# iamgroot42/A-LINK

Measured on AMD Instinct MI355X. Metric: 112x112 face embeddings/sec (IR-ResNet-100 ArcFace, 512-d, L2-normalised), higher is better.
Workload: dtype bf16

## Files before the change

### a-link_amd/csrc/alink_common.h

```cpp
#pragma once
#include <hip/hip_runtime.h>
#include <stdint.h>
#include <stddef.h>
#include <string>

#include "../../include/alink_hip.h"
#include "conv_kernel.h"

namespace alink {

void set_error(const char* fmt, ...);
int  hip_fail(hipError_t e, const char* what, const char* file, int line);

#define ALINK_HIP(call)                                                          \
    do {                                                                         \
        hipError_t e__ = (call);                                                 \
        if (e__ != hipSuccess) return ::alink::hip_fail(e__, #call, __FILE__, __LINE__); \
    } while (0)

#define ALINK_REQUIRE(cond, code, ...)          \
    do {                                        \
        if (!(cond)) {                          \
            ::alink::set_error(__VA_ARGS__);    \
            return (code);                      \
        }                                       \
    } while (0)

static inline int current_device() {
    int d = -1;
    return hipGetDevice(&d) == hipSuccess ? d : -1;
}
static inline int device_of_pointer(const void* p) {
    if (p) {
        hipPointerAttribute_t a;
        if (hipPointerGetAttributes(&a, p) == hipSuccess && a.type == hipMemoryTypeDevice) return a.device;
        (void)hipGetLastError();
    }
    return current_device();
}
struct DeviceGuard {
    int prev = -1;
    bool switched = false;
    explicit DeviceGuard(int dev) {
        if (dev < 0 || hipGetDevice(&prev) != hipSuccess || prev == dev) return;
        switched = hipSetDevice(dev) == hipSuccess;
    }
    ~DeviceGuard() {
        if (switched) (void)hipSetDevice(prev);
    }
    DeviceGuard(const DeviceGuard&) = delete;
    DeviceGuard& operator=(const DeviceGuard&) = delete;
};

typedef __attribute__((ext_vector_type(8))) __bf16   bf16x8;
typedef __attribute__((ext_vector_type(8))) _Float16 f16x8;
typedef __attribute__((ext_vector_type(4))) float    f32x4;
typedef __attribute__((ext_vector_type(16))) float   f32x16;

struct ConvParams {
    const void*  in;
    const void*  wgt;
    const float* bias;
    const float* alpha;
    const void*  resid;
    const void*  dact;
    void*        out;
    const void*  zero;
    const void*  in2;
    int Cin2;
    int in2_compact;
    int N, H, W, Cin, Cout, Ho, Wo, stride, ksz, pad, M;
    int border_cls;
    int splitk;
    int ksteps_per_split;
    int post_relu;
    int fine;
    int stagger;
    int ablate;
    float acc_scale;
    float bias_scale;
    float res_scale;
    int nprod;
    void* stamps;
};

hipError_t launch_conv_igemm(int dtype, const ConvParams& p, hipStream_t stream);
double     conv_flops(const ConvParams& p);

struct StemParams {
    const void*  in;
    const void*  wgt;
    const float* bias;
    const float* alpha;
    void*        out;
    int N, H, W, C0, layout;
    float sub[3], mul;
    int flip;
    float acc_scale, bias_scale;
};
hipError_t launch_stem(int dtype, const StemParams& p, hipStream_t stream);

struct FcFinishParams {
    const float* slabs;
    const float* bias;
    float*       out;
    float*       norms;
    int S, M, E;
    float scale;
    int*  nonfinite;
};
hipError_t launch_fc_finish(const FcFinishParams& p, hipStream_t stream);
hipError_t launch_absmax_f16(const void* x, size_t n_elements, unsigned* out_bits, hipStream_t stream);
hipError_t launch_conv_split_finish(int dtype, const ConvParams& p, const float* slabs, int S, hipStream_t stream);

ConvKernel direct_variant(int ksz, int stride, int pad, int H, int W, int Cin, int Cout);
ConvKernel direct_variant_tiles(int ksz, int stride, int pad, int H, int W, int Cin, int Cout);
ConvKernel linear_variant_x2(int ksz, int stride, int pad, int H, int W, int Cin, int Cout);
hipError_t launch_conv(ConvKernel k, int dtype, const ConvParams& p, hipStream_t st);
hipError_t direct_set_attributes();
ConvKernel linear_variant(int ksz, int stride, int pad, int H, int W, int Cin, int Cout);
ConvKernel c64_variant(int ksz, int stride, int pad, int H, int W, int Cin, int Cout);
ConvKernel s2c64_variant(int ksz, int stride, int pad, int H, int W, int Cin, int Cout);
hipError_t launch_conv3x3_linear(ConvKernel k, int dtype, const ConvParams& p, hipStream_t st);
hipError_t launch_conv3x3_c64(int dtype, const ConvParams& p, hipStream_t st);
hipError_t launch_conv3x3_s2c64(int dtype, const ConvParams& p, hipStream_t st);
hipError_t c64_set_attributes();
hipError_t s2c64_set_attributes();
bool       s2c64_enabled();
hipError_t linear_set_attributes();
hipError_t linear_check_contract();
bool       front_c64_applies(int dtype, int H, int W, int C0, int Cout);
hipError_t front_c64_set_attributes();
hipError_t launch_front_c64(int dtype, const ConvParams& conv1, const StemParams& stem, void* xs, bool slopes_le_1, hipStream_t st);
bool       unit_c64_applies(int dtype, const ConvParams& c1, const ConvParams& c2);
hipError_t unit_c64_set_attributes();
hipError_t launch_unit_c64(int dtype, const ConvParams& c1, const ConvParams& c2, hipStream_t st);
bool       unit1_c64_applies(int dtype, const ConvParams& c1, const StemParams& stem, const ConvParams& c2);
int        unit1_c64_mode();
hipError_t unit1_c64_set_attributes();
hipError_t launch_unit1_c64(int dtype, const ConvParams& c1, const StemParams& stem, const ConvParams& c2, bool slopes_le_1, hipStream_t st);
bool       conv3x3_lat_applies(int dtype, const ConvParams& p);
hipError_t launch_conv3x3_lat(int dtype, const ConvParams& p, hipStream_t stream);
bool       conv_gemm_lat_applies(int dtype, const ConvParams& p);
hipError_t launch_conv_gemm_lat(int dtype, const ConvParams& p, hipStream_t stream);

hipError_t launch_l2norm_bwd(int dtype, const float* g, const float* e, const float* norms, void* dz, int M, int E,
                             hipStream_t st);
hipError_t launch_zero_insert(int dtype, const void* in, void* out, int N, int H, int W, int Ho, int Wo, int C,
                              hipStream_t st);
hipError_t launch_stem_bwd(int dtype, const void* dy0, const void* y0, const float* w, const float* alpha, float* dpix,
                           int N, int H, int W, float mul, int nchw, hipStream_t st);

hipError_t launch_r50_grad_scale(const float* dfeat, int count, int HW, float* scale, hipStream_t st);
hipError_t launch_r50_avgpool_bwd(int dtype, const float* dfeat, const void* y, void* dz, const float* scale, int N, int HW, int C,
                                  hipStream_t st);
hipError_t launch_r50_relu_mask(int dtype, void* g, const void* y, long long count, hipStream_t st);
hipError_t launch_r50_scatter_mask(int dtype, const void* in, const void* y, void* out, int N, int H, int W, int Ho, int Wo, int C,
                                   hipStream_t st);
hipError_t launch_r50_maxpool_bwd(int dtype, const void* y0, const void* pooled, const void* g, void* d0, int N, int H, int W, int C,
                                  int Hp, int Wp, hipStream_t st);
hipError_t launch_r50_stem_bwd(int dtype, const void* d0, const void* wfrag, float* dpix, const float* scale, int N, int H, int W,
                               int Ho, int Wo, int pad_t, int pad_l, int flip, hipStream_t st);
int r50_stem_bwd_max_width();

uint16_t f32_to_bf16_rne(float f);
uint16_t f32_to_f16_rne(float f);

int init_kernels();

__device__ __forceinline__ float relu_keep_nan(float v) { return v < 0.f ? 0.f : v; }
__device__ __forceinline__ float max_keep_nan(float a, float b) { return (a < b || b != b) ? b : a; }

}
#include <map>
#include <string>
#include <vector>
namespace alink {
struct F32Net;
F32Net* f32net_build(const std::map<std::string, std::vector<float>>& raw, const alink_ir_cfg& cfg);
void    f32net_destroy(F32Net* n);
size_t  f32net_workspace_bytes(const F32Net* n, int N);
int     f32net_embed(const F32Net* n, const void* dev_in, int layout, int N, float* dev_out, void* ws, size_t ws_bytes,
                     hipStream_t st);

}
```

### a-link_amd/csrc/conv3x3_linear.hip

```cpp
#include "conv_device.h"

namespace alink {
namespace {

template <int A>
struct IC { static constexpr int a = A; };

constexpr int GPX = 224;
constexpr int TPW = 7;
constexpr int NT = 256;

template <int W, int TCW>
struct Lin {
    static constexpr int BN = 2 * TCW * 16;
    static constexpr int XPIX = GPX + 2 * W + 2;
    static constexpr int XSLOTS = (XPIX * 8 + NT - 1) / NT;
    static constexpr int XBYTES = XSLOTS * NT * 16;
    static constexpr int WOFF = XBYTES;
    static constexpr int WBYTES = BN * 128;
    static constexpr size_t lds_bytes() { return (size_t)WOFF + 2 * WBYTES + 10 * BN * 4; }
    static_assert(GPX % W == 0, "a workgroup covers whole rows");
};

template <typename T, int W, int TCW, int EPI, bool SP, int NP = 3>
__global__ __launch_bounds__(NT, 2) void conv3x3_linear_kernel(const ConvParams p) {
    typedef typename Vec8<T>::type vec8;
    typedef Lin<W, TCW> G;
    constexpr int BN = G::BN, XSLOTS = G::XSLOTS, WBYTES = G::WBYTES, WSLOTS = BN * 8 / NT;
    extern __shared__ __attribute__((aligned(16))) char smem[];

    const int tid = threadIdx.x, lane = tid & 63;
    const int wave = __builtin_amdgcn_readfirstlane(tid >> 6);
    const int wpx = wave >> 1, wco = wave & 1;
    if (p.stagger > 0) {
        __shared__ int s_late;
        if (tid == 0) s_late = (int)(__builtin_amdgcn_s_getreg(6148) & 1u);
        __syncthreads();
        if (s_late)
            for (int i = 0; i < p.stagger; ++i) __builtin_amdgcn_s_sleep(16);
    }
    const int q = lane >> 4, lr = lane & 15;
    const int H = p.H, Cin = p.Cin;
    unsigned long long* const stamps = (EPI == 1 || EPI == 2) ? nullptr : (unsigned long long*)p.stamps;
    unsigned long long refill_cycles = 0;
    if (stamps && tid == 0) stamps[(size_t)blockIdx.x * 8 + 0] = __builtin_amdgcn_s_memtime();
    constexpr int NPH = SP ? NP : 1;
    const int CinP = SP ? 2 * Cin : Cin;
    const int ncc_all = Cin >> 6;
    const int ncc = ncc_all / p.splitk, cc_first = (int)blockIdx.y * ncc;
    const int nk = ncc * 9 * NPH;
    const int K = 9 * CinP;
    const long long totpix = (long long)p.N * H * W;

    const int ntn = p.Cout / BN;
    const int lid = xcd_remap(blockIdx.x, gridDim.x);
    const int tile_n = lid % ntn, grp = lid / ntn;
    const int n0 = tile_n * BN;
    const long long gp0 = (long long)grp * GPX;

    const T* __restrict__ gin = (const T*)p.in;
    const T* __restrict__ gw = (const T*)p.wgt;
    const T* __restrict__ gz = (const T*)p.zero;

    const int xpos0 = tid >> 3;
    const int xc16 = (tid & 7) ^ ((tid >> 4) & 7);
    const long long xgp0 = gp0 - W - 1 + xpos0;
    auto stage_x = [&](int cc, int part = 0) {
        long long x0 = xgp0;
        if (SP) asm volatile("" : "+v"(x0));
#pragma unroll
        for (int i = 0; i < XSLOTS; ++i) {
            const long long gp = x0 + 32 * i;
            const bool ok = xpos0 + 32 * i < G::XPIX && gp >= 0 && gp < totpix;
            const T* src = ok ? gin + ((size_t)gp * CinP + (SP ? 2 * cc + part : cc) * 64 + xc16 * 8) : gz + (lane & 7) * 8;
            dma16(src, smem + (NT * i + wave * 64) * 16);
        }
    };
    const unsigned woff0 = (unsigned)((tid >> 3) * K + (((tid & 7) ^ ((tid >> 4) & 7)) * 8));
    const T* wstep = gw + (size_t)n0 * K + (size_t)cc_first * (SP ? 18 : 9) * 64;
    int wr = 0;
    auto stage_w = [&](int bufoff) {
#pragma unroll
        for (int i = 0; i < WSLOTS; ++i)
            dma16(wstep + (woff0 + (unsigned)(32 * i * K)), smem + G::WOFF + bufoff + (NT * i + wave * 64) * 16);
        if (SP && NP == 1) {
            wstep += wr == 8 ? 10 * 64 : 64;
            wr = wr == 8 ? 0 : wr + 1;
        } else if (SP) {
            wstep += wr == 17 ? -17 * 64 : (wr == 26 ? 10 * 64 : 64);
            wr = wr == 26 ? 0 : wr + 1;
        } else {
            wstep += 64;
        }
    };

    stage_x(cc_first);
    stage_w(0);
    const int ncls = p.border_cls ? 9 : 1;
    constexpr int TBL_TRIPS = (9 * BN + NT - 1) / NT;
    static_assert(BN <= NT, "the slope table is one trip");
    float tbias[TBL_TRIPS], talpha;
#pragma unroll
    for (int k = 0; k < TBL_TRIPS; ++k) {
        const int i = tid + NT * k;
        tbias[k] = p.bias[i < ncls * BN ? (i / BN) * p.Cout + n0 + (i % BN) : 0];
    }
    {
        const float* ap = p.alpha ? p.alpha + n0 + (tid < BN ? tid : 0) : p.bias;
        talpha = *ap;
    }

    const int dl = delta(lr);
    const int xbase = wpx * (TPW * 2048);
    unsigned border = 0;
#pragma unroll
    for (int u = 0; u < TPW; ++u) {
        const int pl = 16 * (wpx * TPW + u) + dl;
        const int col = pl % W;
        const int y = (int)(((unsigned)grp * (unsigned)(GPX / W) + (unsigned)(pl / W)) % (unsigned)W);
        border |= ((y == 0 ? 1u : 0u) | (y == H - 1 ? 2u : 0u) | (col == 0 ? 4u : 0u) | (col == W - 1 ? 8u : 0u)) << (4 * u);
    }
    int wl[2];
    {
        const int rowb = wco * (16 * TCW) + lr;
        const int f = (lr >> 1) & 7;
        wl[0] = G::WOFF + rowb * 128 + (((0 | q) ^ f) << 4);
        wl[1] = G::WOFF + rowb * 128 + (((4 | q) ^ f) << 4);
    }

    f32x4 acc[TCW][TPW];
#pragma unroll
    for (int t = 0; t < TCW; ++t)
#pragma unroll
        for (int u = 0; u < TPW; ++u) acc[t][u] = f32x4{0.f, 0.f, 0.f, 0.f};

    asm volatile("" : "+v"(border));
#pragma unroll
    for (int t = 0; t < TCW; ++t)
#pragma unroll
        for (int u = 0; u < TPW; ++u) asm volatile("" : "+v"(acc[t][u]));

    float* const ebias = (float*)(smem + G::WOFF + 2 * WBYTES);
    float* const ealpha = ebias + 9 * BN;
#pragma unroll
    for (int k = 0; k < TBL_TRIPS; ++k) {
        const int i = tid + NT * k;
        if (i < ncls * BN) ebias[i] = tbias[k] * (SP ? p.bias_scale : 1.f);
    }
    if (p.alpha && tid < BN) ealpha[tid] = talpha;
    wait_then_barrier<0>();
    if (stamps && tid == 0) stamps[(size_t)blockIdx.x * 8 + 1] = __builtin_amdgcn_s_memtime();

    int wtog = 0;
    for (int cc = 0; cc < ncc; ++cc) {
#pragma unroll 1
      for (int ph = 0; ph < NPH; ++ph) {
        auto step = [&](auto tapc) {
            constexpr int tap = decltype(tapc)::a;
            constexpr int ky = tap / 3, kx = tap % 3;
            constexpr unsigned tapbits = (ky == 0 ? 1u : 0u) | (ky == 2 ? 2u : 0u) | (kx == 0 ? 4u : 0u) | (kx == 2 ? 8u : 0u);
            const int t = (cc * NPH + ph) * 9 + tap;
            if (t + 1 < nk) stage_w(wtog ^ WBYTES);
            unsigned bnow = border;
            int sdl = dl;
            asm volatile("" : "+v"(bnow), "+v"(sdl));
            const int spos = sdl + ky * W + kx;
            const int xt0 = xbase + spos * 128 + ((q ^ ((spos >> 1) & 7)) << 4);
            const int xt1 = xt0 ^ 64;
#pragma unroll
            for (int ks = 0; ks < 2; ++ks) {
                vec8 wf[TCW], pf[TPW];
#pragma unroll
                for (int tt = 0; tt < TCW; ++tt) wf[tt] = *(const vec8*)(smem + (wl[ks] + wtog) + tt * 2048);
#pragma unroll
                for (int u = 0; u < TPW; ++u) {
                    const unsigned t = tapbits ? (bnow & (tapbits << (4 * u))) : 0u;
                    const unsigned far = 4 * u < 18 ? t << (18 - (4 * u < 18 ? 4 * u : 0)) : t;
                    pf[u] = *(const vec8*)(smem + ((ks ? xt1 : xt0) + (int)far) + 2048 * u);
                }
#pragma unroll
                for (int tt = 0; tt < TCW; ++tt)
#pragma unroll
                    for (int u = 0; u < TPW; ++u) acc[tt][u] = mfma16<T>(wf[tt], pf[u], acc[tt][u]);
            }
            wait_then_barrier<0>();
            wtog ^= WBYTES;
        };
        step(IC<0>{}); step(IC<1>{}); step(IC<2>{});
        step(IC<3>{}); step(IC<4>{}); step(IC<5>{});
        step(IC<6>{}); step(IC<7>{}); step(IC<8>{});
        const bool next_chunk = ph == NPH - 1;
        if (next_chunk ? cc + 1 < ncc : ph == 1) {
            const unsigned long long t0 = stamps ? __builtin_amdgcn_s_memtime() : 0ull;
            if (next_chunk) stage_x(cc_first + cc + 1, 0);
            else            stage_x(cc_first + cc, 1);
            wait_then_barrier<0>();
            if (stamps) refill_cycles += __builtin_amdgcn_s_memtime() - t0;
        }
      }
    }
    if (stamps && tid == 0) {
        stamps[(size_t)blockIdx.x * 8 + 2] = __builtin_amdgcn_s_memtime();
        stamps[(size_t)blockIdx.x * 8 + 4] = refill_cycles;
        stamps[(size_t)blockIdx.x * 8 + 5] = (unsigned long long)(ncc - 1);
    }

    constexpr int CPL = TCW * 4;
    const int wbase = wco * (16 * TCW);
    auto chan_t = [&](int t) { return wbase + (TCW == 4 ? 32 * (t >> 1) + 8 * q + 4 * (t & 1) : 8 * q + 4 * t); };
    auto chan_h = [&](int h) { return wbase + (TCW == 4 ? 32 * h + 8 * q : 8 * q); };
    if (SP ? EPI == 3 : (EPI == 0 && p.splitk > 1)) {
        float* slab = (float*)p.out + (size_t)blockIdx.y * (size_t)totpix * p.Cout;
#pragma unroll
        for (int u = 0; u < TPW; ++u) {
            const long long gp = gp0 + 16 * (wpx * TPW + u) + dl;
            if (gp < totpix) {
#pragma unroll
                for (int t = 0; t < TCW; ++t) *(f32x4*)(slab + (size_t)gp * p.Cout + n0 + chan_t(t)) = acc[t][u];
            }
        }
        return;
    }
    if constexpr (SP) {
        size_t off[TPW];
        bool ok[TPW];
#pragma unroll
        for (int u = 0; u < TPW; ++u) {
            const long long gp = gp0 + 16 * (wpx * TPW + u) + dl;
            ok[u] = gp < totpix;
            off[u] = (size_t)(ok[u] ? gp : 0) * (2 * p.Cout);
            const unsigned b4 = (border >> (4 * u)) & 15u;
            const int rc = (b4 & 1u) ? 0 : ((b4 & 2u) ? 2 : 1);
            const int ccl = (b4 & 4u) ? 0 : ((b4 & 8u) ? 2 : 1);
            const int cls = p.border_cls ? rc * 3 + ccl : 0;
#pragma unroll
            for (int t = 0; t < TCW; ++t) {
                const f32x4 b = *(const f32x4*)(ebias + cls * BN + chan_t(t));
#pragma unroll
                for (int j = 0; j < 4; ++j) acc[t][u][j] = fmaf(acc[t][u][j], p.acc_scale, b[j]);
            }
        }
        if (EPI == 1 || (EPI == 0 && p.alpha)) {
#pragma unroll
            for (int t = 0; t < TCW; ++t) {
                const f32x4 a4 = *(const f32x4*)(ealpha + chan_t(t));
#pragma unroll
                for (int u = 0; u < TPW; ++u)
#pragma unroll
                    for (int j = 0; j < 4; ++j) acc[t][u][j] = acc[t][u][j] > 0.f ? acc[t][u][j] : acc[t][u][j] * a4[j];
            }
        }
        int so[CPL / 8];
#pragma unroll
        for (int h = 0; h < CPL / 8; ++h) so[h] = ((n0 + chan_h(h)) >> 6) * 128 + ((n0 + chan_h(h)) & 63);
        if (EPI != 1 && p.resid) {
            const T* r = (const T*)p.resid;
#pragma unroll
            for (int part = 0; part < 2; ++part) {
                vec8 res[TPW][CPL / 8];
#pragma unroll
                for (int u = 0; u < TPW; ++u)
#pragma unroll
                    for (int h = 0; h < CPL / 8; ++h) res[u][h] = *(const vec8*)(r + off[u] + so[h] + 64 * part);
#pragma unroll
                for (int u = 0; u < TPW; ++u)
#pragma unroll
                    for (int h = 0; h < CPL / 8; ++h)
#pragma unroll
                        for (int i = 0; i < 8; ++i)
                            acc[2 * h + (i >> 2)][u][i & 3] = fmaf((float)res[u][h][i], p.res_scale, acc[2 * h + (i >> 2)][u][i & 3]);
            }
        }
#pragma unroll
        for (int u = 0; u < TPW; ++u) {
            if (!ok[u]) continue;
#pragma unroll
            for (int h = 0; h < CPL / 8; ++h) {
                vec8 o8, l8;
#pragma unroll
                for (int i = 0; i < 8; ++i) {
                    float v = acc[2 * h + (i >> 2)][u][i & 3];
                    if (EPI == 0 && p.post_relu) v = relu_keep_nan(v);
                    o8[i] = (T)v;
                    l8[i] = (T)(v - (float)o8[i]);
                }
                *(vec8*)((T*)p.out + off[u] + so[h]) = o8;
                *(vec8*)((T*)p.out + off[u] + so[h] + 64) = l8;
            }
        }
        return;
    }
    auto epilogue16 = [&](auto fullc) {
        constexpr bool FULL = decltype(fullc)::a != 0;
        size_t off[TPW];
        bool ok[TPW];
        int cls[TPW];
#pragma unroll
        for (int u = 0; u < TPW; ++u) {
            const long long gp = gp0 + 16 * (wpx * TPW + u) + dl;
            ok[u] = FULL || gp < totpix;
            off[u] = (size_t)(FULL || ok[u] ? gp : 0) * p.Cout + n0;
            const unsigned b4 = (border >> (4 * u)) & 15u;
            const int rc = (b4 & 1u) ? 0 : ((b4 & 2u) ? 2 : 1);
            const int ccl = (b4 & 4u) ? 0 : ((b4 & 8u) ? 2 : 1);
            cls[u] = p.border_cls ? rc * 3 + ccl : 0;
        }
        vec8 res[TPW][CPL / 8];
        const T* extra = EPI == 1 ? (const T*)nullptr : (const T*)((EPI == 0 && p.dact) ? p.dact : p.resid);
        if (EPI == 2 || (EPI == 0 && extra)) {
#pragma unroll
            for (int u = 0; u < TPW; ++u)
#pragma unroll
                for (int h = 0; h < CPL / 8; ++h) res[u][h] = *(const vec8*)(extra + off[u] + chan_h(h));
            __builtin_amdgcn_sched_barrier(0);
        }
        if (stamps) {
            asm volatile("s_waitcnt vmcnt(0)" ::: "memory");
            if (tid == 0) stamps[(size_t)blockIdx.x * 8 + 6] = __builtin_amdgcn_s_memtime();
        }
#pragma unroll
        for (int u = 0; u < TPW; ++u) {
            float v[CPL];
#pragma unroll
            for (int t = 0; t < TCW; ++t) {
                const f32x4 b4 = *(const f32x4*)(ebias + cls[u] * BN + chan_t(t));
#pragma unroll
                for (int j = 0; j < 4; ++j) v[4 * t + j] = acc[t][u][j] + b4[j];
            }
            if (EPI == 0 && p.dact) {
#pragma unroll
                for (int t = 0; t < TCW; ++t) {
                    const f32x4 a4 = *(const f32x4*)(ealpha + chan_t(t));
#pragma unroll
                    for (int j = 0; j < 4; ++j) v[4 * t + j] *= (float)res[u][(4 * t + j) / 8][(4 * t + j) % 8] > 0.f ? 1.f : a4[j];
                }
            } else {
                if (EPI == 1 || (EPI == 0 && p.alpha)) {
#pragma unroll
                    for (int t = 0; t < TCW; ++t) {
                        const f32x4 a4 = *(const f32x4*)(ealpha + chan_t(t));
#pragma unroll
                        for (int j = 0; j < 4; ++j) v[4 * t + j] = v[4 * t + j] > 0.f ? v[4 * t + j] : v[4 * t + j] * a4[j];
                    }
                }
                if (EPI == 2 || (EPI == 0 && p.resid)) {
#pragma unroll
                    for (int h = 0; h < CPL / 8; ++h)
#pragma unroll
                        for (int i = 0; i < 8; ++i) v[8 * h + i] += (float)res[u][h][i];
                }
            }
            if (EPI == 0 && p.post_relu) {
#pragma unroll
                for (int i = 0; i < CPL; ++i) v[i] = relu_keep_nan(v[i]);
            }
            if (FULL || ok[u]) {
#pragma unroll
                for (int h = 0; h < CPL / 8; ++h) {
                    vec8 o8;
#pragma unroll
                    for (int i = 0; i < 8; ++i) o8[i] = (T)v[8 * h + i];
                    *(vec8*)((T*)p.out + off[u] + chan_h(h)) = o8;
                }
            }
        }
    };
    if (gp0 + GPX <= totpix) epilogue16(IC<1>{});
    else                     epilogue16(IC<0>{});
    if (stamps && tid == 0) {
        stamps[(size_t)blockIdx.x * 8 + 7] = __builtin_amdgcn_s_memtime();
        asm volatile("s_waitcnt vmcnt(0)" ::: "memory");
        stamps[(size_t)blockIdx.x * 8 + 3] = __builtin_amdgcn_s_memtime();
    }
}

bool g_generic_epilogue = false;

template <typename T, int W, int TCW, bool SP = false>
hipError_t launch_one(const ConvParams& p, hipStream_t st) {
    typedef Lin<W, TCW> G;
    const long long totpix = (long long)p.N * p.H * W;
    const long long groups = (totpix + GPX - 1) / GPX;
    const long long nwg = groups * (p.Cout / G::BN);
    if (nwg <= 0 || nwg >= (1ll << 31)) return hipErrorInvalidValue;
    const dim3 grid((unsigned)nwg, (unsigned)p.splitk);
    if (SP) {
        if (p.dact) return hipErrorInvalidValue;
        if (p.nprod == 1) {
            if (p.splitk > 1) hipLaunchKernelGGL((conv3x3_linear_kernel<T, W, TCW, 3, SP, 1>), grid, dim3(NT), G::lds_bytes(), st, p);
            else              hipLaunchKernelGGL((conv3x3_linear_kernel<T, W, TCW, 0, SP, 1>), grid, dim3(NT), G::lds_bytes(), st, p);
            return hipGetLastError();
        }
        const bool plain_sp = p.splitk == 1 && !p.post_relu && !p.stamps && !g_generic_epilogue;
        if (p.splitk > 1) hipLaunchKernelGGL((conv3x3_linear_kernel<T, W, TCW, 3, SP>), grid, dim3(NT), G::lds_bytes(), st, p);
        else if (plain_sp && p.alpha && !p.resid)
            hipLaunchKernelGGL((conv3x3_linear_kernel<T, W, TCW, 1, SP>), grid, dim3(NT), G::lds_bytes(), st, p);
        else if (plain_sp && !p.alpha && p.resid)
            hipLaunchKernelGGL((conv3x3_linear_kernel<T, W, TCW, 2, SP>), grid, dim3(NT), G::lds_bytes(), st, p);
        else              hipLaunchKernelGGL((conv3x3_linear_kernel<T, W, TCW, 0, SP>), grid, dim3(NT), G::lds_bytes(), st, p);
        return hipGetLastError();
    }
    const bool plain = p.splitk == 1 && !p.dact && !p.post_relu && !p.stamps && !g_generic_epilogue;
    if (plain && p.alpha && !p.resid)
        hipLaunchKernelGGL((conv3x3_linear_kernel<T, W, TCW, 1, false>), grid, dim3(NT), G::lds_bytes(), st, p);
    else if (plain && !p.alpha && p.resid)
        hipLaunchKernelGGL((conv3x3_linear_kernel<T, W, TCW, 2, false>), grid, dim3(NT), G::lds_bytes(), st, p);
    else
        hipLaunchKernelGGL((conv3x3_linear_kernel<T, W, TCW, 0, false>), grid, dim3(NT), G::lds_bytes(), st, p);
    return hipGetLastError();
}
template <typename T, int W, int TCW>
hipError_t set_attr_one() {
    const int lds = (int)Lin<W, TCW>::lds_bytes();
    hipError_t e = hipFuncSetAttribute((const void*)conv3x3_linear_kernel<T, W, TCW, 0, false>, hipFuncAttributeMaxDynamicSharedMemorySize, lds);
    if (e == hipSuccess) e = hipFuncSetAttribute((const void*)conv3x3_linear_kernel<T, W, TCW, 1, false>, hipFuncAttributeMaxDynamicSharedMemorySize, lds);
    if (e == hipSuccess) e = hipFuncSetAttribute((const void*)conv3x3_linear_kernel<T, W, TCW, 2, false>, hipFuncAttributeMaxDynamicSharedMemorySize, lds);
    return e;
}
template <int W, int TCW>
hipError_t set_attr_sp() {
    hipError_t e = hipFuncSetAttribute((const void*)conv3x3_linear_kernel<_Float16, W, TCW, 0, true>,
                                       hipFuncAttributeMaxDynamicSharedMemorySize, (int)Lin<W, TCW>::lds_bytes());
    if (e == hipSuccess)
        e = hipFuncSetAttribute((const void*)conv3x3_linear_kernel<_Float16, W, TCW, 3, true>,
                                hipFuncAttributeMaxDynamicSharedMemorySize, (int)Lin<W, TCW>::lds_bytes());
    if (e == hipSuccess)
        e = hipFuncSetAttribute((const void*)conv3x3_linear_kernel<_Float16, W, TCW, 1, true>,
                                hipFuncAttributeMaxDynamicSharedMemorySize, (int)Lin<W, TCW>::lds_bytes());
    if (e == hipSuccess)
        e = hipFuncSetAttribute((const void*)conv3x3_linear_kernel<_Float16, W, TCW, 2, true>,
                                hipFuncAttributeMaxDynamicSharedMemorySize, (int)Lin<W, TCW>::lds_bytes());
    if (e == hipSuccess)
        e = hipFuncSetAttribute((const void*)conv3x3_linear_kernel<_Float16, W, TCW, 0, true, 1>,
                                hipFuncAttributeMaxDynamicSharedMemorySize, (int)Lin<W, TCW>::lds_bytes());
    if (e == hipSuccess)
        e = hipFuncSetAttribute((const void*)conv3x3_linear_kernel<_Float16, W, TCW, 3, true, 1>,
                                hipFuncAttributeMaxDynamicSharedMemorySize, (int)Lin<W, TCW>::lds_bytes());
    return e;
}

int g_linear_mode = 31;

}

extern "C" void alink_debug_set_linear(int mode) { g_linear_mode = mode; }
extern "C" void alink_debug_set_generic_epilogue(int on) { g_generic_epilogue = on != 0; }

namespace {
__global__ void lds_oob_probe_kernel(float* out) {
    __shared__ __attribute__((aligned(16))) float buf[256];
    for (int i = threadIdx.x; i < 256; i += 64) buf[i] = 1.0f + i;
    __syncthreads();
    const unsigned base = (unsigned)(size_t)(__attribute__((address_space(3))) float*)buf;
    const int lane = threadIdx.x;
    unsigned bits;
    if (lane < 10) {
        bits = 1u << (18 + lane);
    } else if (lane < 55) {
        int k = lane - 10, a = 18;
        while (k >= 27 - a) { k -= 27 - a; ++a; }
        bits = (1u << a) | (1u << (a + 1 + k));
    } else {
        bits = 0x0FFC0000u >> (lane - 55) & 0x0FFC0000u;
    }
    const unsigned far = base + (lane & 15) * 16u + bits, near = base + (lane & 3) * 16u;
    f32x4 a0, a1, b;
    asm volatile("ds_read_b128 %0, %3\n\tds_read_b128 %1, %3 offset:12288\n\tds_read_b128 %2, %4\n\ts_waitcnt lgkmcnt(0)"
                 : "=&v"(a0), "=&v"(a1), "=&v"(b) : "v"(far), "v"(near) : "memory");
    *(f32x4*)(out + lane * 8) = a0;
    *(f32x4*)(out + lane * 8 + 4) = a1;
    if (lane == 0) *(f32x4*)(out + 512) = b;
}
constexpr int PROBE_FLOATS = 516;
bool g_contract_ok[64] = {};
}
hipError_t linear_check_contract() {
    const int dev = current_device();
    float* d = nullptr;
    hipError_t e = hipMalloc((void**)&d, PROBE_FLOATS * sizeof(float));
    if (e != hipSuccess) return e;
    float h[PROBE_FLOATS];
    for (int i = 0; i < PROBE_FLOATS; ++i) h[i] = 7.f;
    e = hipMemcpy(d, h, sizeof(h), hipMemcpyHostToDevice);
    if (e == hipSuccess) {
        hipLaunchKernelGGL(lds_oob_probe_kernel, dim3(1), dim3(64), 0, (hipStream_t)0, d);
        e = hipGetLastError();
    }
    if (e == hipSuccess) e = hipMemcpy(h, d, sizeof(h), hipMemcpyDeviceToHost);
    (void)hipFree(d);
    if (e != hipSuccess) return e;
    bool ok = h[512] == 1.f && h[513] == 2.f && h[514] == 3.f && h[515] == 4.f;
    for (int i = 0; i < 512; ++i) ok = ok && h[i] == 0.f;
    if (dev >= 0 && dev < 64) g_contract_ok[dev] = ok;
    return hipSuccess;
}

extern "C" int alink_debug_lds_oob_probe(float* dev_out516, void* stream) {
    DeviceGuard dg(device_of_pointer(dev_out516));
    hipLaunchKernelGGL(lds_oob_probe_kernel, dim3(1), dim3(64), 0, (hipStream_t)stream, dev_out516);
    return hipGetLastError() == hipSuccess ? 0 : -1;
}
extern "C" int alink_debug_linear_contract_ok(void) {
    const int dev = current_device();
    return dev >= 0 && dev < 64 && g_contract_ok[dev] ? 1 : 0;
}

ConvKernel linear_variant(int ksz, int stride, int pad, int H, int W, int Cin, int Cout) {
    if (ksz != 3 || stride != 1 || pad != 1 || H != W || Cin % 64) return ConvKernel::Igemm;
    const int dev = current_device();
    if (dev < 0 || dev >= 64 || !g_contract_ok[dev]) return ConvKernel::Igemm;
    if ((g_linear_mode & 4) && W == 14 && Cout % 128 == 0) return ConvKernel::Linear14;
    if ((g_linear_mode & 2) && W == 28 && Cout % 128 == 0) return ConvKernel::Linear28;
    if ((g_linear_mode & 1) && W == 56 && Cout % 64 == 0) return ConvKernel::Linear56;
    if ((g_linear_mode & 8) && W == 7 && Cout % 128 == 0) return ConvKernel::Linear7;
    return ConvKernel::Igemm;
}
ConvKernel linear_variant_x2(int ksz, int stride, int pad, int H, int W, int Cin, int Cout) {
    const ConvKernel k = linear_variant(ksz, stride, pad, H, W, Cin, Cout);
    if (k != ConvKernel::Igemm) return k;
    if (ksz != 3 || stride != 1 || pad != 1 || H != W || Cin % 64) return ConvKernel::Igemm;
    const int dev = current_device();
    if (dev < 0 || dev >= 64 || !g_contract_ok[dev]) return ConvKernel::Igemm;
    if ((g_linear_mode & 16) && W == 112 && Cout % 64 == 0) return ConvKernel::Linear112;
    return ConvKernel::Igemm;
}

hipError_t linear_set_attributes() {
    hipError_t e;
#define A(T)                                                              \
    if ((e = set_attr_one<T, 14, 4>()) != hipSuccess) return e;           \
    if ((e = set_attr_one<T, 28, 4>()) != hipSuccess) return e;           \
    if ((e = set_attr_one<T, 56, 2>()) != hipSuccess) return e;           \
    if ((e = set_attr_one<T, 7, 4>()) != hipSuccess) return e;            \
    if ((e = set_attr_one<T, 14, 2>()) != hipSuccess) return e;           \
    if ((e = set_attr_one<T, 28, 2>()) != hipSuccess) return e;           \
    if ((e = set_attr_one<T, 7, 2>()) != hipSuccess) return e;
    A(__bf16) A(_Float16)
#undef A
#define B(W_, TCW_) if ((e = set_attr_sp<W_, TCW_>()) != hipSuccess) return e;
    B(14, 4) B(28, 4) B(56, 2) B(7, 4) B(14, 2) B(28, 2) B(7, 2) B(112, 2)
#undef B
    return hipSuccess;
}

hipError_t launch_conv3x3_linear(ConvKernel k, int dtype, const ConvParams& p, hipStream_t st) {
    if (p.ksz != 3 || p.stride != 1 || p.pad != 1 || p.H != p.W) return hipErrorInvalidValue;
    if (conv3x3_lat_applies(dtype, p)) return launch_conv3x3_lat(dtype, p, st);
    if (p.splitk < 1 || (p.Cin / 64) % p.splitk) return hipErrorInvalidValue;
    if ((long long)p.N * p.H * p.W * p.Cin * (dtype == ALINK_DT_F16X2 ? 2 : 1) >= (1ll << 31)) return hipErrorInvalidValue;
#define L(W_, TCW_) (dtype == ALINK_DT_BF16 ? launch_one<__bf16, W_, TCW_>(p, st) : (dtype == ALINK_DT_F16X2 ? launch_one<_Float16, W_, TCW_, true>(p, st) : launch_one<_Float16, W_, TCW_>(p, st)))
    if (p.fine) {
        switch (k) {
            case ConvKernel::Linear14: return p.W == 14 ? L(14, 2) : hipErrorInvalidValue;
            case ConvKernel::Linear28: return p.W == 28 ? L(28, 2) : hipErrorInvalidValue;
            case ConvKernel::Linear7:  return p.W == 7 ? L(7, 2) : hipErrorInvalidValue;
            default: break;
        }
    }
    switch (k) {
        case ConvKernel::Linear14:  return p.W == 14 ? L(14, 4) : hipErrorInvalidValue;
        case ConvKernel::Linear28:  return p.W == 28 ? L(28, 4) : hipErrorInvalidValue;
        case ConvKernel::Linear56:  return p.W == 56 ? L(56, 2) : hipErrorInvalidValue;
        case ConvKernel::Linear7:   return p.W == 7 ? L(7, 4) : hipErrorInvalidValue;
        case ConvKernel::Linear112: return p.W == 112 && dtype == ALINK_DT_F16X2 ? launch_one<_Float16, 112, 2, true>(p, st) : hipErrorInvalidValue;
        default: break;
    }
#undef L
    return hipErrorInvalidValue;
}

}
```

### include/alink_hip_debug.h

```cpp
#ifndef ALINK_HIP_DEBUG_H
#define ALINK_HIP_DEBUG_H

#include <stddef.h>

#ifdef __cplusplus
extern "C" {
#endif

void alink_debug_set_linear(int mode);
void alink_debug_set_generic_epilogue(int on);
void alink_debug_set_direct(int on);
void alink_debug_set_pair(int on);
void alink_debug_set_c64(int on);
void alink_debug_set_s2direct(int on);
void alink_debug_set_fuse_stem(int on);
void alink_debug_set_fuse_unit(int mode);
void alink_debug_set_fuse_unit1(int mode);
void alink_debug_set_fuse_shortcut(int on);
void alink_debug_set_dma(int on);
void alink_debug_set_fine_max(int n);
void alink_debug_set_sibling_aware(int on);
void alink_debug_set_latency_form(int max_pixels);
void alink_debug_set_latency_tiles(int form);
void alink_debug_set_stagger(int n);
void alink_debug_set_shard_stagger(int on);

void alink_debug_set_tiny_step(int on);
void alink_debug_set_mini_step(int on);
void alink_debug_set_head_bf16_mfma(int on);

void alink_debug_set_smallres_overlap(int on);
void alink_debug_set_smallres_one_update(int on);

void alink_debug_set_stop_after(int n);
void alink_debug_set_profile_reps(int n);
void alink_debug_set_ablate(int a);
void alink_debug_set_stamps(void* dev_u64);
int alink_debug_lds_oob_probe(float* dev_out516, void* stream);
int alink_debug_linear_contract_ok(void);


struct alink_resnet50;
struct alink_backbone;
int alink_debug_resnet50_grad_cache_info(const struct alink_resnet50* r, int n_images, int index, size_t* byte_offset, int* H,
                                         int* W, int* C, char* name_buf, int name_len);
int alink_debug_backbone_grad_cache_info(const struct alink_backbone* bb, int n_images, int index, size_t* byte_offset, int* H,
                                         int* W, int* C, char* name_buf, int name_len);

#ifdef __cplusplus
}
#endif
#endif
```

Before: 48640.

## Issue activation refill early inside last tap to overlap with MFMAs

In the linear 3x3 conv kernel, the last tap (tap 8) now loads both k-slices of activation fragments into registers first. It then waits for those LDS reads, places a barrier, and starts the next activation staging (stage_x) before running the remaining MFMAs. This replaces the separate refill-plus-barrier step after the tap loop, so the global-to-LDS refill overlaps with compute and one barrier per phase is removed. The cost is higher register pressure from holding two fragment sets, and reordering risk around LDS reuse. The behaviour is controlled by a new early_refill parameter that is on by default.

```diff
diff --git a/a-link_amd/csrc/alink_common.h b/a-link_amd/csrc/alink_common.h
--- a/a-link_amd/csrc/alink_common.h
+++ b/a-link_amd/csrc/alink_common.h
@@ -76,6 +76,7 @@
     int post_relu;
     int fine;
     int stagger;
+    int early_refill;
     int ablate;
     float acc_scale;
     float bias_scale;
diff --git a/a-link_amd/csrc/conv3x3_linear.hip b/a-link_amd/csrc/conv3x3_linear.hip
--- a/a-link_amd/csrc/conv3x3_linear.hip
+++ b/a-link_amd/csrc/conv3x3_linear.hip
@@ -9,6 +9,12 @@
 constexpr int GPX = 224;
 constexpr int TPW = 7;
 constexpr int NT = 256;
+
+template <typename V>
+__device__ __forceinline__ void reads_back_then_barrier(const V (&p0)[TPW], const V (&p1)[TPW]) {
+    asm volatile("s_waitcnt lgkmcnt(0)\n\ts_barrier" ::"v"(p0[0]), "v"(p0[1]), "v"(p0[2]), "v"(p0[3]), "v"(p0[4]), "v"(p0[5]), "v"(p0[6]),
+                 "v"(p1[0]), "v"(p1[1]), "v"(p1[2]), "v"(p1[3]), "v"(p1[4]), "v"(p1[5]), "v"(p1[6]) : "memory");
+}
 
 template <int W, int TCW>
 struct Lin {
@@ -151,10 +157,19 @@
     wait_then_barrier<0>();
     if (stamps && tid == 0) stamps[(size_t)blockIdx.x * 8 + 1] = __builtin_amdgcn_s_memtime();
 
+    const int early_form = p.early_refill;
     int wtog = 0;
     for (int cc = 0; cc < ncc; ++cc) {
 #pragma unroll 1
       for (int ph = 0; ph < NPH; ++ph) {
+        const bool next_chunk = ph == NPH - 1;
+        const bool refill = next_chunk ? cc + 1 < ncc : ph == 1;
+        const bool early = early_form != 0 && refill;
+        auto refill_x = [&]() {
+            int cn = next_chunk ? cc_first + cc + 1 : cc_first + cc;
+            if (!SP) asm volatile("" : "+s"(cn));
+            stage_x(cn, next_chunk ? 0 : 1);
+        };
         auto step = [&](auto tapc) {
             constexpr int tap = decltype(tapc)::a;
             constexpr int ky = tap / 3, kx = tap % 3;
@@ -167,21 +182,51 @@
             const int spos = sdl + ky * W + kx;
             const int xt0 = xbase + spos * 128 + ((q ^ ((spos >> 1) & 7)) << 4);
             const int xt1 = xt0 ^ 64;
-#pragma unroll
-            for (int ks = 0; ks < 2; ++ks) {
-                vec8 wf[TCW], pf[TPW];
+            auto frags_w = [&](int ks, vec8 (&wf)[TCW]) {
 #pragma unroll
                 for (int tt = 0; tt < TCW; ++tt) wf[tt] = *(const vec8*)(smem + (wl[ks] + wtog) + tt * 2048);
+            };
+            auto frags_x = [&](int ks, vec8 (&pf)[TPW]) {
 #pragma unroll
                 for (int u = 0; u < TPW; ++u) {
                     const unsigned t = tapbits ? (bnow & (tapbits << (4 * u))) : 0u;
                     const unsigned far = 4 * u < 18 ? t << (18 - (4 * u < 18 ? 4 * u : 0)) : t;
                     pf[u] = *(const vec8*)(smem + ((ks ? xt1 : xt0) + (int)far) + 2048 * u);
                 }
+            };
+            auto mfmas = [&](const vec8 (&wf)[TCW], const vec8 (&pf)[TPW], int u0, int u1) {
 #pragma unroll
                 for (int tt = 0; tt < TCW; ++tt)
 #pragma unroll
-                    for (int u = 0; u < TPW; ++u) acc[tt][u] = mfma16<T>(wf[tt], pf[u], acc[tt][u]);
+                    for (int u = u0; u < u1; ++u) acc[tt][u] = mfma16<T>(wf[tt], pf[u], acc[tt][u]);
+            };
+            if constexpr (tap == 8) {
+                vec8 wf0[TCW], pf0[TPW], wf1[TCW], pf1[TPW];
+                frags_w(0, wf0);
+                frags_x(0, pf0);
+                frags_x(1, pf1);
+                __builtin_amdgcn_sched_barrier(0);
+                if (early) {
+                    const unsigned long long t0 = stamps ? __builtin_amdgcn_s_memtime() : 0ull;
+                    reads_back_then_barrier(pf0, pf1);
+                    if (stamps) refill_cycles += __builtin_amdgcn_s_memtime() - t0;
+                    refill_x();
+                }
+                mfmas(wf0, pf0, 0, 4);
+                __builtin_amdgcn_sched_barrier(0);
+                frags_w(1, wf1);
+                __builtin_amdgcn_sched_barrier(0);
+                mfmas(wf0, pf0, 4, TPW);
+                mfmas(wf1, pf1, 0, TPW);
+                __builtin_amdgcn_sched_barrier(0);
+            } else {
+#pragma unroll
+                for (int ks = 0; ks < 2; ++ks) {
+                    vec8 wf[TCW], pf[TPW];
+                    frags_w(ks, wf);
+                    frags_x(ks, pf);
+                    mfmas(wf, pf, 0, TPW);
+                }
             }
             wait_then_barrier<0>();
             wtog ^= WBYTES;
@@ -189,11 +234,9 @@
         step(IC<0>{}); step(IC<1>{}); step(IC<2>{});
         step(IC<3>{}); step(IC<4>{}); step(IC<5>{});
         step(IC<6>{}); step(IC<7>{}); step(IC<8>{});
-        const bool next_chunk = ph == NPH - 1;
-        if (next_chunk ? cc + 1 < ncc : ph == 1) {
+        if (refill && !early) {
             const unsigned long long t0 = stamps ? __builtin_amdgcn_s_memtime() : 0ull;
-            if (next_chunk) stage_x(cc_first + cc + 1, 0);
-            else            stage_x(cc_first + cc, 1);
+            refill_x();
             wait_then_barrier<0>();
             if (stamps) refill_cycles += __builtin_amdgcn_s_memtime() - t0;
         }
@@ -375,10 +418,13 @@
 }
 
 bool g_generic_epilogue = false;
+int g_early_refill = 1;
 
 template <typename T, int W, int TCW, bool SP = false>
-hipError_t launch_one(const ConvParams& p, hipStream_t st) {
+hipError_t launch_one(const ConvParams& p_in, hipStream_t st) {
     typedef Lin<W, TCW> G;
+    ConvParams p = p_in;
+    p.early_refill = g_early_refill;
     const long long totpix = (long long)p.N * p.H * W;
     const long long groups = (totpix + GPX - 1) / GPX;
     const long long nwg = groups * (p.Cout / G::BN);
@@ -445,6 +491,7 @@
 
 extern "C" void alink_debug_set_linear(int mode) { g_linear_mode = mode; }
 extern "C" void alink_debug_set_generic_epilogue(int on) { g_generic_epilogue = on != 0; }
+extern "C" void alink_debug_set_early_refill(int on) { g_early_refill = on != 0 ? 1 : 0; }
 
 namespace {
 __global__ void lds_oob_probe_kernel(float* out) {
diff --git a/include/alink_hip_debug.h b/include/alink_hip_debug.h
--- a/include/alink_hip_debug.h
+++ b/include/alink_hip_debug.h
@@ -23,6 +23,7 @@
 void alink_debug_set_latency_form(int max_pixels);
 void alink_debug_set_latency_tiles(int form);
 void alink_debug_set_stagger(int n);
+void alink_debug_set_early_refill(int on);
 void alink_debug_set_shard_stagger(int on);
 
 void alink_debug_set_tiny_step(int on);
```

New measurement: 49230, median of 6. 1.01x the previous value.
